# HPCForge/Bubbleformer

Measured on AMD Instinct MI355X. Metric: train samples/sec, FiLMAViT 16x192x192x4ch, bs=8 per GPU, higher is better.
Workload: dtype bf16; 1 GPU; FiLMAViT-small (E=384, 6 heads, 12 blocks, P=16, 9 fluid params) fwd + relative-L2 loss + bwd + AdamW, 4-field 16x192x192 clips, batch 8 per GPU (BASELINE.json configs[1]); global_batch=8, parallelism=dp1

## Files before the change

bubbleformer_amd/_lib.py:

```python
import ctypes as C
import os
import subprocess

_HERE = os.path.dirname(os.path.abspath(__file__))
LIB_PATH = os.path.join(_HERE, "libbubbleformer_hip.so")
CSRC = os.path.join(_HERE, "csrc")

BF_DTYPE_F32, BF_DTYPE_BF16 = 0, 1
BF_LAY_KC, BF_LAY_XC = 0, 1
BF_PRO_NONE, BF_PRO_AFFINE, BF_PRO_AFFINE_GELU, BF_PRO_GELU = 0, 1, 2, 3
BF_AUX_NONE, BF_AUX_ADD, BF_AUX_DGELU = 0, 1, 2
BF_OUT_STORE, BF_OUT_STORE_F32, BF_OUT_ATOMIC_F32 = 0, 1, 2
BF_MAX_STAGES = 5
BF_LOSS_LIMBS = 5

vp, fp, i32, i64, f32 = C.c_void_p, C.c_void_p, C.c_int32, C.c_int64, C.c_float


class Operand(C.Structure):
    _fields_ = [("p", vp), ("ld", i64), ("layout", i32), ("seglen", i32), ("segstride", i64), ("gw", i32), ("gh", i32),
                ("gc", i32), ("pro", i32), ("sc", fp), ("sh", fp), ("rows_per_frame", i32), ("nch", i32)]


class Epilogue(C.Structure):
# ... 4 lines not shown

class Dims(C.Structure):
    _fields_ = [(n, i32) for n in ("dtype", "B", "T", "h", "w", "E", "heads", "attn_scale", "feat_scale", "patch", "cin",
                                   "cout", "nfluid")]


TEMPORAL_FIELDS = ("gamma", "attn_scale_factor", "norm1_w", "norm1_b", "norm2_w", "norm2_b", "input_head_w", "input_head_b",
                   "output_head_w", "output_head_b", "qnorm_w", "qnorm_b", "knorm_w", "knorm_b", "rel_pos_emb")
SPATIAL_FIELDS = ("gamma_att", "gamma_mlp", "attn_scale_factor_x", "attn_scale_factor_y", "low_freq_scalar",
                  "high_freq_scalar", "norm1_w", "norm1_b", "norm2_w", "norm2_b", "input_head_w", "input_head_b",
                  "output_head_w", "output_head_b", "qnorm_w", "qnorm_b", "knorm_w", "knorm_b", "rel_pos_emb", "fc1_w", "fc1_b",
                  "fc2_w", "fc2_b", "mlp_norm_w", "mlp_norm_b")


class TemporalParams(C.Structure):
    _fields_ = [(n, fp) for n in TEMPORAL_FIELDS]


class SpatialParams(C.Structure):
    _fields_ = [(n, fp) for n in SPATIAL_FIELDS]


class FrameNorm(C.Structure):
    _fields_ = [("w", fp), ("b", fp), ("g", fp), ("gdiv", i32), ("mean", fp), ("rstd", fp), ("sc", fp), ("sh", fp), ("resid", vp), ("out", vp)]


class EmbedParams(C.Structure):
    _fields_ = [("conv_w", fp * BF_MAX_STAGES), ("in_w", fp * BF_MAX_STAGES), ("in_b", fp * BF_MAX_STAGES), ("film_ln_w", fp),
                ("film_ln_b", fp), ("film_w", fp), ("film_b", fp)]


class DebedParams(C.Structure):
    _fields_ = [("conv_w", fp * BF_MAX_STAGES), ("in_w", fp * BF_MAX_STAGES), ("in_b", fp * BF_MAX_STAGES)]


class ConvSrc(C.Structure):
    _fields_ = [("p", vp), ("C", i32), ("nchw", i32), ("f32", i32)]


class ConvGeo(C.Structure):
    _fields_ = [(n, i32) for n in ("F", "Hi", "Wi", "Ho", "Wo", "kh", "kw", "stride", "pad")]


BF_CONV_PRO_NONE, BF_CONV_PRO_AFFINE_GELU, BF_CONV_PRO_GELU = 0, 1, 2

STAGE_DONE_FN = C.CFUNCTYPE(None, C.c_int, C.c_void_p)
P = C.POINTER
SIGNATURES = {
    "bf_last_error": (C.c_char_p, []),
    "bf_abi_version": (C.c_int, []),
    "bf_prof_enable": (None, [C.c_int]),
    "bf_debug_force_generic_attn": (None, [C.c_int]),
    "bf_debug_tokred_fold": (None, [C.c_int]),
    "bf_side_defer": (None, [C.c_int]),
    "bf_prep_stages": (C.c_int, [C.POINTER(Dims), C.c_int, C.POINTER(C.c_int32), C.POINTER(vp), C.POINTER(vp), C.POINTER(vp), vp]),
    "bf_stage_prepared": (None, [C.c_int]),
    "bf_trunk_train_fwd": (C.c_int, [C.POINTER(Dims), C.c_int, C.POINTER(C.c_int32), C.POINTER(vp), C.POINTER(vp), C.POINTER(vp), C.POINTER(vp), vp,
                                     C.POINTER(vp), vp, vp]),
    "bf_trunk_train_bwd": (C.c_int, [C.POINTER(Dims), C.c_int, C.POINTER(C.c_int32), C.POINTER(vp), C.POINTER(vp), C.POINTER(vp), C.POINTER(vp),
                                     C.POINTER(vp), vp, C.POINTER(vp), vp, C.POINTER(vp), vp, vp, vp, vp, vp]),
    "bf_field_stats_ws_doubles": (i64, [C.c_int]),
    "bf_field_stats": (C.c_int, [fp, vp, vp, C.c_int, vp, vp, vp]),
    "bf_stage_chain_next": (C.c_int, [C.POINTER(Dims), C.c_int, vp, vp]),
    "bf_stage_next_scale": (C.c_int, [fp, C.c_int]),
    "bf_gemm_fwd_frames": (C.c_int, [C.c_int, C.c_int, C.c_int, C.c_int, vp, i64, vp, i64, fp, fp, fp, fp, C.c_int, vp, vp, C.c_int,
                                     C.POINTER(FrameNorm), C.POINTER(FrameNorm), vp]),
    "bf_trunk_eval_weights_bytes": (i64, [C.POINTER(Dims), C.c_int, C.POINTER(C.c_int32)]),
    "bf_trunk_eval_prepare": (C.c_int, [C.POINTER(Dims), C.c_int, C.POINTER(C.c_int32), C.POINTER(vp), vp, vp]),
    "bf_trunk_eval_fwd": (C.c_int, [C.POINTER(Dims), C.c_int, C.POINTER(C.c_int32), C.POINTER(vp), vp, vp, vp, vp, vp]),
    "bf_frame_linear": (C.c_int, [C.c_int, C.c_int, C.c_int, C.c_int, C.c_int, vp, i64, vp, i64, fp, fp, fp, fp, fp, vp, i64, C.c_int, fp, fp, fp,
                                  vp, i64, fp, fp, vp, i64, vp]),
    "bf_side_join": (C.c_int, [vp]),
    "bf_prof_report": (C.c_int, [C.c_char_p, C.c_int]),
    "bf_gemm": (C.c_int, [C.c_int, C.c_int, C.c_int, C.c_int, P(Operand), P(Operand), P(Epilogue), C.c_int, vp]),
    "bf_gemm_tokred": (C.c_int, [C.c_int, C.c_int, C.c_int, i64, vp, i64, vp, i64, fp, C.c_int, fp, fp, i64, vp]),
    "bf_gemm_tokred_ws_floats": (i64, [C.c_int, C.c_int, i64]),
    "bf_gemm_inbwd_frames": (C.c_int, [C.c_int, C.c_int, C.c_int, C.c_int, vp, i64, vp, i64, vp, vp, vp, C.c_int, fp, fp, fp, fp, fp, C.c_int, vp]),
    "bf_gemm_inbwd_frames_chain": (C.c_int, [C.c_int, C.c_int, C.c_int, C.c_int, vp, i64, vp, i64, vp, vp, vp, C.c_int, fp, fp, fp, fp, fp, C.c_int,
                                             vp, vp, fp, fp, fp, fp, C.c_int, fp, vp]),
    "bf_in_stats": (C.c_int, [C.c_int, vp, C.c_int, C.c_int, C.c_int, fp, fp, fp, C.c_int, fp, fp, fp, fp, fp, fp, vp]),
    "bf_in_ws_floats": (i64, [C.c_int, C.c_int, C.c_int, C.c_int]),
    "bf_affine_apply": (C.c_int, [C.c_int, vp, vp, fp, fp, vp, i64, C.c_int, C.c_int, vp]),
    "bf_in_bwd": (C.c_int, [C.c_int, vp, vp, vp, vp, C.c_int, C.c_int, C.c_int, fp, fp, fp, fp, fp, C.c_int, C.c_int, fp, fp,
                            fp, fp, fp, vp]),
    "bf_colsum": (C.c_int, [C.c_int, vp, i64, C.c_int, fp, fp, vp]),
    "bf_attn_axial_fwd": (C.c_int, [C.c_int, vp, vp, i64, C.c_int, C.c_int, C.c_int, C.c_int, fp, fp, fp, fp, fp, fp, fp, vp]),
    "bf_attn_axial_norm_fwd": (C.c_int, [C.c_int, vp, vp, vp, i64, C.c_int, C.c_int, C.c_int, C.c_int, fp, fp, fp, fp, fp, fp, fp, fp, fp, fp, fp, fp,
                                         fp, vp]),
    "bf_attn_fwd": (C.c_int, [C.c_int, vp, vp, i64, C.c_int, i64, i64, i64, i64, C.c_int, C.c_int, fp, fp, fp, fp, fp, fp, f32,
                              C.c_int, vp]),
    "bf_attn_bwd": (C.c_int, [C.c_int, vp, vp, vp, i64, C.c_int, i64, i64, i64, i64, C.c_int, C.c_int, fp, fp, fp, fp, fp, fp,
                              fp, fp, fp, fp, fp, fp, f32, C.c_int, fp, i64, vp]),
    "bf_im2col_nchw": (C.c_int, [C.c_int, fp, vp, C.c_int, C.c_int, C.c_int, C.c_int, C.c_int, vp]),
    "bf_col2im_nchw": (C.c_int, [C.c_int, vp, fp, C.c_int, C.c_int, C.c_int, C.c_int, C.c_int, vp]),
    "bf_pm2nchw": (C.c_int, [fp, fp, fp, fp, C.c_int, C.c_int, C.c_int, C.c_int, C.c_int, vp]),
    "bf_debed_last_bwd": (C.c_int, [C.c_int, fp, fp, fp, fp, fp, vp, vp, vp, C.c_int, C.c_int, C.c_int, C.c_int, C.c_int, C.c_int, vp]),
    "bf_debed_last_bwd_norm": (C.c_int, [C.c_int, fp, fp, fp, fp, fp, vp, vp, vp, fp, fp, fp, fp, vp, fp, fp, C.c_int, C.c_int, C.c_int, C.c_int, C.c_int,
                                         C.c_int, fp, C.c_int64, vp]),
    "bf_gather_gemm": (C.c_int, [C.c_int, vp, vp, C.c_int, fp, fp, vp, C.c_int, C.c_int, C.c_int, C.c_int, C.c_int, vp]),
    "bf_scatter_gemm": (C.c_int, [C.c_int, vp, vp, C.c_int, fp, fp, vp, fp, C.c_int, C.c_int, C.c_int, C.c_int, C.c_int, vp]),
    "bf_gather_wgrad_ws_floats": (C.c_int64, [C.c_int, C.c_int, C.c_int]),
    "bf_gather_wgrad": (C.c_int, [C.c_int, vp, vp, fp, fp, fp, fp, fp, C.c_int, C.c_int, C.c_int, C.c_int, C.c_int, C.c_int, fp, C.c_int64, vp]),
    "bf_gather_gemm_rebuilt": (C.c_int, [C.c_int, vp, vp, vp, C.c_int, fp, fp, vp, C.c_int, C.c_int, C.c_int, C.c_int, C.c_int, vp]),
    "bf_gather_wgrad_rebuilt": (C.c_int, [C.c_int, vp, vp, vp, fp, fp, fp, C.c_int, C.c_int, C.c_int, C.c_int, C.c_int, C.c_int, fp, C.c_int64, vp]),
    "bf_stage_chain_head": (C.c_int, [vp, vp, vp]),
    "bf_stage_chain_tail": (C.c_int, [vp, vp, C.c_int]),
# ... 118 lines not shown
```

bubbleformer_amd/csrc/bf_common.h:

```cpp
#pragma once
#include <hip/hip_runtime.h>
#include <stdint.h>
#include <math.h>

#include "../../include/bubbleformer_hip.h"

typedef __bf16 bf16;
typedef __attribute__((ext_vector_type(8))) __bf16 bf16x8;
typedef __attribute__((ext_vector_type(4))) __bf16 bf16x4;
typedef __attribute__((ext_vector_type(4))) short s16x4;
typedef __attribute__((ext_vector_type(4))) float f32x4;

#define BF_WAVE 64
#define BF_IN_EPS 1e-5f

#define BF_CHECK_LAUNCH()                                   \
    do {                                                    \
        hipError_t e__ = hipGetLastError();                 \
        if (e__ != hipSuccess) return bf_fail(e__, __FILE__, __LINE__); \
    } while (0)
#define BF_REQUIRE(cond, msg)                                \
    do {                                                     \
        if (!(cond)) return bf_fail_msg(msg, __FILE__, __LINE__); \
    } while (0)
// ... 40 lines not shown
    bool& flag() { int dev = 0; (void)hipGetDevice(&dev); return done[(dev >= 0 && dev < 64) ? dev : 0]; }
};
template <class T> struct BfPerDevice {
    T tab[64] = {};
    T& get() { int dev = 0; (void)hipGetDevice(&dev); return tab[(dev >= 0 && dev < 64) ? dev : 0]; }
};
int bf_fail(hipError_t e, const char* file, int line);
int bf_fail_msg(const char* msg, const char* file, int line);
int bf_decline(const char* msg);

__device__ __forceinline__ float to_f(float x) { return x; }
__device__ __forceinline__ float to_f(bf16 x) { return (float)x; }
template <typename T> __device__ __forceinline__ T from_f(float x);
template <> __device__ __forceinline__ float from_f<float>(float x) { return x; }
template <> __device__ __forceinline__ bf16 from_f<bf16>(float x) { return (bf16)x; }

template <typename T> struct Chunk;
template <> struct Chunk<float> {
    static constexpr int N = 4;
    float4 raw;
    __device__ __forceinline__ void load(const float* p) { raw = *reinterpret_cast<const float4*>(p); }
    __device__ __forceinline__ void store(float* p) const { *reinterpret_cast<float4*>(p) = raw; }
    __device__ __forceinline__ void zero() { raw = make_float4(0.f, 0.f, 0.f, 0.f); }
    __device__ __forceinline__ float get(int i) const { return i == 0 ? raw.x : i == 1 ? raw.y : i == 2 ? raw.z : raw.w; }
    __device__ __forceinline__ void set(int i, float v) { if (i == 0) raw.x = v; else if (i == 1) raw.y = v; else if (i == 2) raw.z = v; else raw.w = v; }
};
template <> struct Chunk<bf16> {
    static constexpr int N = 8;
    bf16x8 raw;
    __device__ __forceinline__ void load(const bf16* p) { raw = *reinterpret_cast<const bf16x8*>(p); }
    __device__ __forceinline__ void store(bf16* p) const { *reinterpret_cast<bf16x8*>(p) = raw; }
    __device__ __forceinline__ void zero() { for (int i = 0; i < 8; ++i) raw[i] = (bf16)0.f; }
    __device__ __forceinline__ float get(int i) const { return (float)raw[i]; }
    __device__ __forceinline__ void set(int i, float v) { raw[i] = (bf16)v; }
};

__device__ __forceinline__ float erf_fast(float x) {
    const float ax = fabsf(x);
    const float t = __builtin_amdgcn_rcpf(1.0f + 0.3275911f * ax);
    const float poly = t * (0.254829592f + t * (-0.284496736f + t * (1.421413741f + t * (-1.453152027f + t * 1.061405429f))));
    const float r = 1.0f - poly * __expf(-ax * ax);
    return copysignf(r, x);
}
__device__ __forceinline__ float gelu_f(float x) { return 0.5f * x * (1.0f + erf_fast(x * 0.70710678118654752440f)); }
__device__ __forceinline__ float dgelu_f(float x) {
    const float ax = fabsf(x) * 0.70710678118654752440f;
    const float t = __builtin_amdgcn_rcpf(1.0f + 0.3275911f * ax);
    const float poly = t * (0.254829592f + t * (-0.284496736f + t * (1.421413741f + t * (-1.453152027f + t * 1.061405429f))));
    const float e = __expf(-0.5f * x * x);
    const float cdf = 0.5f * (1.0f + copysignf(1.0f - poly * e, x));
    return cdf + x * (0.39894228040143267794f * e);
}

__device__ __forceinline__ float phi_fast(float x) {
    const float xc = fminf(fmaxf(x, -4.0f), 4.0f), u = xc * xc;
    float r = -1.520480094e-09f;
    r = r * u + 1.180964698e-07f; r = r * u - 4.014221545e-06f; r = r * u + 7.960997465e-05f; r = r * u - 1.041295800e-03f;
    r = r * u + 9.641715296e-03f; r = r * u - 6.614117438e-02f; r = r * u + 3.988329119e-01f;
    return 0.5f + xc * r;
}
__device__ __forceinline__ float gelu_fast(float x) { return x * phi_fast(x); }
__device__ __forceinline__ float dgelu_fast(float x) {
    const float xc = fminf(fmaxf(x, -4.0f), 4.0f), u = xc * xc;
    float r = 9.387459194e-10f;
    r = r * u - 7.941240515e-08f; r = r * u + 2.950722870e-06f; r = r * u - 6.380590451e-05f; r = r * u + 8.975979855e-04f;
    r = r * u - 8.669717964e-03f; r = r * u + 5.833777581e-02f; r = r * u - 2.646917422e-01f; r = r * u + 7.975648121e-01f;
    return 0.5f + xc * r;
}

template <typename T> __device__ __forceinline__ float gelu_t(float x) { if constexpr (sizeof(T) == 2) return gelu_fast(x); else return gelu_f(x); }
template <typename T> __device__ __forceinline__ float dgelu_t(float x) { if constexpr (sizeof(T) == 2) return dgelu_fast(x); else return dgelu_f(x); }

template <class T> __device__ __forceinline__ T wave_sum(T v) {
#pragma unroll
    for (int o = 32; o > 0; o >>= 1) v += __shfl_xor(v, o, 64);
    return v;
}
__device__ __forceinline__ float wave_max(float v) {
#pragma unroll
    for (int o = 32; o > 0; o >>= 1) v = fmaxf(v, __shfl_xor(v, o, 64));
    return v;
}

static inline int bf_cdiv(long a, long b) { return (int)((a + b - 1) / b); }
static inline size_t bf_esize(int dtype) { return dtype == BF_DTYPE_BF16 ? 2 : 4; }
```

bubbleformer_amd/csrc/gemm_stream.hip:

```cpp
#include "gemm_common.h"
#include <stdio.h>
#include <stdlib.h>
#include <algorithm>

namespace {
using namespace bfgemm;

constexpr int BM = 256, BNB = 128, BK = 64;
constexpr int CHUNK = BNB * BK;
constexpr int ACHUNK = BM * BK;
constexpr int NSLOT = 2;

struct StreamArgs {
    const bf16* A; long lda; const bf16* W; long ldw; bf16* C; long ldc;
    const float* bias; const float* colscale; const float* colshift; const float* rowscale; int rpg;
    int aux_mode; const bf16* aux; long ld_aux; bf16* gelu_out;
    int KS, mt, nb, ng;
    int mh, hunit;
    int stagger;
    int dbg;
};

__device__ __forceinline__ void wait_vm_n(int n) {
    if (n >= 16) { wait_vm<16>(); return; }
    switch (n) {
        case 0: wait_vm<0>(); break;   case 1: wait_vm<1>(); break;   case 2: wait_vm<2>(); break;   case 3: wait_vm<3>(); break;
        case 4: wait_vm<4>(); break;   case 5: wait_vm<5>(); break;   case 6: wait_vm<6>(); break;   case 7: wait_vm<7>(); break;
        case 8: wait_vm<8>(); break;   case 9: wait_vm<9>(); break;   case 10: wait_vm<10>(); break; case 11: wait_vm<11>(); break;
        case 12: wait_vm<12>(); break; case 13: wait_vm<13>(); break; case 14: wait_vm<14>(); break; default: wait_vm<15>(); break;
    }
}
__device__ __forceinline__ void gload16(uint4& dst, const void* p) { asm volatile("global_load_dwordx4 %0, %1, off" : "=v"(dst) : "v"(p) : "memory"); }

__device__ __forceinline__ void gload4(float& dst, const void* p) { asm volatile("global_load_dword %0, %1, off" : "=v"(dst) : "v"(p) : "memory"); }

template <int AUX, bool GELU2, bool CS>
__global__ void __launch_bounds__(512) stream_gemm_kernel(StreamArgs a) {
    extern __shared__ __attribute__((aligned(16))) char smem[];
    bf16* Bres = reinterpret_cast<bf16*>(smem);
    bf16* ring = Bres + (size_t)a.KS * CHUNK;
    const int KS = a.KS;
    const int tid = threadIdx.x, lane = tid & 63, wave = __builtin_amdgcn_readfirstlane(tid >> 6);
    const int wm = wave >> 1, wn = wave & 1;

    const int xl = blockIdx.x & 7, j = blockIdx.x >> 3, wpx = gridDim.x >> 3;
    const int tpx = wpx / a.nb;
    if (j >= tpx * a.nb) return;
    const int team = xl * tpx + j / a.nb, nteams = 8 * tpx;
    const int grp = team % a.ng, rank = team / a.ng, gteams = (nteams - grp + a.ng - 1) / a.ng;
    const int c_nb = grp * a.nb + j % a.nb;
    const int h_beg = a.hunit * (int)((long)(a.mh / a.hunit) * rank / gteams), h_end = a.hunit * (int)((long)(a.mh / a.hunit) * (rank + 1) / gteams);
    if (h_beg >= h_end) return;
    const int ntile = (h_end - h_beg + 1) >> 1;
    const bool odd_run = (h_end - h_beg) & 1;
    const int total_steps = ntile * KS;

    long roffA[4], roffB[2];
#pragma unroll
    for (int t = 0; t < 4; ++t) {
        const int r = 8 * (wave * 4 + t) + (lane >> 3);
        roffA[t] = (long)r * a.lda + 8 * ((lane & 7) ^ ((r >> 1) & 7));
    }
#pragma unroll
    for (int t = 0; t < 2; ++t) {
        const int r = 8 * (wave * 2 + t) + (lane >> 3);
        roffB[t] = (long)r * a.ldw + 8 * ((lane & 7) ^ ((r >> 1) & 7));
    }
    const unsigned lds0 = lds_addr(smem);
    const unsigned ldsB = __builtin_amdgcn_readfirstlane(lds0 + (unsigned)wave * 2048u);
    const unsigned ldsA = __builtin_amdgcn_readfirstlane(lds0 + (unsigned)KS * (unsigned)(CHUNK * 2) + (unsigned)wave * 4096u);

    int issued = 0;
    int i_ks = 0, i_left = total_steps, i_slot = 0;
    const bf16* i_row = a.A + (long)((a.dbg & 2) ? 0 : h_beg) * (BM / 2) * a.lda;
    auto issue_A = [&]() {
        const unsigned dst = ldsA + (unsigned)i_slot * (unsigned)(ACHUNK * 2);
        if (!(odd_run && i_left <= KS && wave >= 4)) {
#pragma unroll
            for (int t = 0; t < 4; ++t) glds16(i_row + roffA[t] + i_ks * BK, dst + t * 1024u);
            issued += 4;
        }
        i_slot ^= 1;
        --i_left;
        if (++i_ks == KS) { i_ks = 0; if (!(a.dbg & 2)) i_row += (long)BM * a.lda; }
    };

    const int li = lane & 15, lg = lane >> 4;
    const int c8 = wn * 64 + (lg & 1) * 16 + (lg >> 1) * 8;
    float e_bias[2][8], e_cs[2][CS ? 8 : 1], e_ch[2][CS ? 8 : 1];
    {
#pragma unroll
        for (int pp = 0; pp < 2; ++pp)
#pragma unroll
            for (int q = 0; q < 8; ++q) {
                const int n = c_nb * BNB + c8 + 32 * pp + q;
                e_bias[pp][q] = a.bias ? a.bias[n] : 0.f;
                if constexpr (CS) { e_cs[pp][q] = a.colscale ? a.colscale[n] : 1.f; e_ch[pp][q] = a.colscale ? a.colshift[n] : 0.f; }
            }
#pragma unroll
        for (int pp = 0; pp < 2; ++pp)
#pragma unroll
            for (int q = 0; q < 8; ++q) {
                asm volatile("" : "+v"(e_bias[pp][q]));
                if constexpr (CS) { asm volatile("" : "+v"(e_cs[pp][q])); asm volatile("" : "+v"(e_ch[pp][q])); }
            }
    }

    int bmark[6];
    const bf16* w0 = a.W + (long)c_nb * BNB * a.ldw;
    auto load_W = [&](int kb) {
#pragma unroll
        for (int t = 0; t < 2; ++t) glds16(w0 + roffB[t] + kb * BK, ldsB + (unsigned)kb * (unsigned)(CHUNK * 2) + t * 1024u);
        issued += 2;
        return issued;
    };
    bmark[0] = load_W(0);
    issue_A();
    int mark = issued, mark_next = issued;
    bmark[1] = load_W(1);
    const bool pre1 = i_left > 0;
    if (pre1) { issue_A(); mark_next = issued; }
#pragma unroll
    for (int kb = 2; kb < 6; ++kb) bmark[kb] = kb < KS ? load_W(kb) : issued;
    bool first_tile = true;

    f32x4 acc[4][4];
    uint4 auxr[4][2];
    float rsr[4] = {1.f, 1.f, 1.f, 1.f};
    const bool has_rs = CS && a.rowscale != nullptr;
    int aux_mark = 0;
    int slot = 0;
    auto run_tile = [&](int tt) __attribute__((always_inline)) {
        const int m0 = h_beg * (BM / 2) + tt * BM;
#pragma unroll
        for (int i = 0; i < 4; ++i)
#pragma unroll
            for (int jn = 0; jn < 4; ++jn) acc[i][jn] = f32x4{0.f, 0.f, 0.f, 0.f};
        for (int ks = 0; ks < KS; ++ks) {
            int need = mark;
            if (first_tile) { const int bm = ks == 0 ? bmark[0] : ks == 1 ? bmark[1] : ks == 2 ? bmark[2] : ks == 3 ? bmark[3] : ks == 4 ? bmark[4] : bmark[5]; need = max(need, bm); }
            if (!(a.dbg & 1)) wait_vm_n(issued - need);
            asm volatile("s_waitcnt lgkmcnt(0)" ::: "memory");
            __builtin_amdgcn_s_barrier();
            if (ks == 0) {
                if constexpr (AUX != BF_AUX_NONE) {
#pragma unroll
                    for (int i = 0; i < 4; ++i)
#pragma unroll
                        for (int pp = 0; pp < 2; ++pp)
                            gload16(auxr[i][pp], a.aux + (long)(m0 + wm * 64 + i * 16 + li) * a.ld_aux + c_nb * BNB + c8 + 32 * pp);
                    issued += 8;
                }
                if (has_rs) {
#pragma unroll
                    for (int i = 0; i < 4; ++i) gload4(rsr[i], a.rowscale + (m0 + wm * 64 + i * 16 + li) / a.rpg);
                    issued += 4;
                }
                aux_mark = issued;
            }
            const bool late = a.stagger && wave >= 4;
            const bool skip = first_tile && ks == 0 && pre1;
            if (!late && !skip) { if (i_left > 0 && !(a.dbg & 32)) issue_A(); mark_next = issued; }
            const bf16* cA = ring + (size_t)slot * ACHUNK;
            const bf16* cB = Bres + (size_t)ks * CHUNK;
            if (!(a.dbg & 4))
#pragma unroll
            for (int kk = 0; kk < BK; kk += 32) {
                if (kk == 32 && late && !skip) { if (i_left > 0 && !(a.dbg & 32)) issue_A(); mark_next = issued; }
                bf16x8 fa[4], fb[4];
#pragma unroll
                for (int i = 0; i < 4; ++i) fa[i] = frag_bf16<false, BK>(cA, wm * 64 + i * 16, kk, lane);
#pragma unroll
                for (int jn = 0; jn < 4; ++jn) fb[jn] = frag_bf16<false, BK>(cB, wn * 64 + jn * 16, kk, lane);
#pragma unroll
                for (int i = 0; i < 4; ++i)
#pragma unroll
                    for (int jn = 0; jn < 4; ++jn) acc[i][jn] = __builtin_amdgcn_mfma_f32_16x16x32_bf16(fb[jn], fa[i], acc[i][jn], 0, 0, 0);
            }
            slot ^= 1;
            mark = mark_next;
        }
        first_tile = false;
        if (AUX != BF_AUX_NONE || has_rs) {
            wait_vm_n(issued - aux_mark);
            if constexpr (AUX != BF_AUX_NONE) {
#pragma unroll
                for (int i = 0; i < 4; ++i)
#pragma unroll
                    for (int pp = 0; pp < 2; ++pp) asm volatile("" : "+v"(auxr[i][pp].x), "+v"(auxr[i][pp].y), "+v"(auxr[i][pp].z), "+v"(auxr[i][pp].w));
            }
            if constexpr (CS) {
#pragma unroll
                for (int i = 0; i < 4; ++i) asm volatile("" : "+v"(rsr[i]));
            }
            __builtin_amdgcn_sched_barrier(0);
        }
#pragma unroll
        for (int i = 0; i < 4; ++i) {
            const int m = m0 + wm * 64 + i * 16 + li;
#pragma unroll
            for (int pp = 0; pp < 2; ++pp) {
                float v[8];
#pragma unroll
                for (int r = 0; r < 4; ++r) {
                    typedef __attribute__((ext_vector_type(2))) unsigned u32x2;
                    const u32x2 sw = __builtin_amdgcn_permlane16_swap(__float_as_uint(acc[i][2 * pp][r]), __float_as_uint(acc[i][2 * pp + 1][r]), false, false);
                    v[r] = __uint_as_float(sw[0]); v[4 + r] = __uint_as_float(sw[1]);
                }
                if constexpr (AUX == BF_AUX_ADD) {
                    const bf16x8 ax = __builtin_bit_cast(bf16x8, auxr[i][pp]);
#pragma unroll
                    for (int q = 0; q < 8; ++q) {
                        float cs_ = 1.f, ch_ = 0.f;
                        if constexpr (CS) { cs_ = e_cs[pp][q]; ch_ = e_ch[pp][q]; }
                        v[q] = epi_lin_add(v[q], e_bias[pp][q], cs_, ch_, has_rs ? rsr[i] : 1.f, CS, (float)ax[q]);
                    }
                } else {
#pragma unroll
                    for (int q = 0; q < 8; ++q) {
                        float cs_ = 1.f, ch_ = 0.f;
                        if constexpr (CS) { cs_ = e_cs[pp][q]; ch_ = e_ch[pp][q]; }
                        v[q] = epi_lin(v[q], e_bias[pp][q], cs_, ch_, has_rs ? rsr[i] : 1.f, CS);
                    }
                    if constexpr (AUX == BF_AUX_DGELU) {
                        const bf16x8 ax = __builtin_bit_cast(bf16x8, auxr[i][pp]);
#pragma unroll
                        for (int q = 0; q < 8; ++q) v[q] = v[q] * dgelu_fast((float)ax[q]);
                    }
                }
                bf16x8 o;
#pragma unroll
                for (int q = 0; q < 8; ++q) o[q] = (bf16)v[q];
                const long off = (long)m * a.ldc + c_nb * BNB + c8 + 32 * pp;
                if (a.dbg & 16) asm volatile("" :: "v"(o)); else
                if (!(a.dbg & 8)) *reinterpret_cast<bf16x8*>(a.C + off) = o;
                if constexpr (GELU2) {
                    bf16x8 g8;
#pragma unroll
                    for (int q = 0; q < 8; ++q) g8[q] = (bf16)gelu_fast(v[q]);
                    *reinterpret_cast<bf16x8*>(a.gelu_out + off) = g8;
                }
            }
        }
        issued += GELU2 ? 16 : 8;
    };
    const int nfull = odd_run ? ntile - 1 : ntile;
    for (int tt = 0; tt < nfull; ++tt) run_tile(tt);
    if (odd_run) {
        if (wave < 4) run_tile(ntile - 1);
        else
            for (int ks = 0; ks < KS; ++ks) {
                wait_vm<0>();
                asm volatile("s_waitcnt lgkmcnt(0)" ::: "memory");
                __builtin_amdgcn_s_barrier();
            }
    }
}


constexpr int PSLOT = (ACHUNK + CHUNK) * 2;
constexpr int PNSLOT = 3;

__device__ __forceinline__ void wait_vm_wide(int n) {
    if (n < 16) { wait_vm_n(n); return; }
    if (n >= 40) { wait_vm<40>(); return; }
    switch ((n - 16) >> 2) {
        case 0: wait_vm<16>(); break; case 1: wait_vm<20>(); break; case 2: wait_vm<24>(); break;
        case 3: wait_vm<28>(); break; case 4: wait_vm<32>(); break; default: wait_vm<36>(); break;
    }
}

template <int AUX, bool GELU2, bool CS>
__global__ void __launch_bounds__(512) stream_pp_kernel(StreamArgs a) {
    extern __shared__ __attribute__((aligned(16))) char smem[];
    const int KS = a.KS;
    const int tid = threadIdx.x, lane = tid & 63, wave = __builtin_amdgcn_readfirstlane(tid >> 6);
    const int wm = wave >> 1, wn = wave & 1;
    const bool late = wave >= 4;

    const int xl = blockIdx.x & 7, j = blockIdx.x >> 3, wpx = gridDim.x >> 3;
    const int tpx = wpx / a.nb;
    if (j >= tpx * a.nb) return;
    const int team = xl * tpx + j / a.nb, nteams = 8 * tpx;
    const int grp = team % a.ng, rank = team / a.ng, gteams = (nteams - grp + a.ng - 1) / a.ng;
    const int c_nb = grp * a.nb + j % a.nb;
    const int t_beg = (int)((long)a.mt * rank / gteams), t_end = (int)((long)a.mt * (rank + 1) / gteams);
    if (t_beg >= t_end) return;
    const int total_steps = (t_end - t_beg) * KS;

    long roffA[4], roffB[2];
#pragma unroll
    for (int t = 0; t < 4; ++t) {
        const int r = 8 * (wave * 4 + t) + (lane >> 3);
        roffA[t] = (long)r * a.lda + 8 * ((lane & 7) ^ ((r >> 1) & 7));
    }
#pragma unroll
    for (int t = 0; t < 2; ++t) {
        const int r = 8 * (wave * 2 + t) + (lane >> 3);
        roffB[t] = (long)r * a.ldw + 8 * ((lane & 7) ^ ((r >> 1) & 7));
    }
    const unsigned lds0 = lds_addr(smem);
    const unsigned ldsA = __builtin_amdgcn_readfirstlane(lds0 + (unsigned)wave * 4096u);
    const unsigned ldsB = __builtin_amdgcn_readfirstlane(lds0 + (unsigned)(ACHUNK * 2) + (unsigned)wave * 2048u);
    const bf16* w0 = a.W + (long)c_nb * BNB * a.ldw;

    int issued = 0;
    int i_ks = 0, i_left = total_steps, i_slot = 0;
    const bf16* i_row = a.A + (long)t_beg * BM * a.lda;
    auto issue_lo = [&]() {
// ... 153 lines not shown
                        float cs_ = 1.f, ch_ = 0.f;
                        if constexpr (CS) { cs_ = e_cs[pp][q]; ch_ = e_ch[pp][q]; }
                        v[q] = epi_lin(v[q], e_bias[pp][q], cs_, ch_, has_rs ? rsr[i] : 1.f, CS);
                    }
                    if constexpr (AUX == BF_AUX_DGELU) {
                        const bf16x8 ax = __builtin_bit_cast(bf16x8, auxr[i][pp]);
#pragma unroll
                        for (int q = 0; q < 8; ++q) v[q] = v[q] * dgelu_fast((float)ax[q]);
                    }
                }
                bf16x8 o;
#pragma unroll
                for (int q = 0; q < 8; ++q) o[q] = (bf16)v[q];
                const long off = (long)m * a.ldc + c_nb * BNB + c8 + 32 * pp;
                *reinterpret_cast<bf16x8*>(a.C + off) = o;
                if constexpr (GELU2) {
                    bf16x8 g8;
#pragma unroll
                    for (int q = 0; q < 8; ++q) g8[q] = (bf16)gelu_fast(v[q]);
                    *reinterpret_cast<bf16x8*>(a.gelu_out + off) = g8;
                }
            }
        }
        issued += GELU2 ? 16 : 8;
    }
}


int num_cus() {
    static const int n = []() {
        int dev = 0; hipDeviceProp_t p;
        if (hipGetDevice(&dev) != hipSuccess || hipGetDeviceProperties(&p, dev) != hipSuccess || p.multiProcessorCount < 8) return 256;
        return p.multiProcessorCount;
    }();
    return n;
}

bool team_split(int NB, int mt, int wpx, int* nb, int* ng) {
    static const int force = bf_knob("BF_STREAM_GROUPS", 0);
    int best = 0, best_cost = 0;
    for (int g = 1; g <= NB; ++g) {
        if (NB % g || NB / g > wpx || (force > 0 && g != force)) continue;
        const int nteams = 8 * (wpx / (NB / g));
        if (nteams < g) continue;
        const int fewest = nteams / g;
        const int cost = (mt + fewest - 1) / fewest;
        if (!best || cost < best_cost) { best = g; best_cost = cost; }
    }
    if (!best) return false;
    *ng = best; *nb = NB / best;
    return true;
}

}

int bf_gemm_stream_try(int M, int N, int K, const bf_operand* A, const bf_operand* B, const bf_epilogue* E, hipStream_t st) {
    static const int enabled = bf_knob("BF_GEMM_STREAM", 1);
    if (!enabled) return 1;
    if (A->layout != BF_LAY_KC || B->layout != BF_LAY_KC || A->pro != BF_PRO_NONE || B->pro != BF_PRO_NONE) return 1;
    if (A->gw > 0 || A->seglen > 0 || B->gw > 0 || B->seglen > 0 || E->gw > 0 || E->seglen > 0) return 1;
    if (E->out_mode != BF_OUT_STORE || E->colsum) return 1;
    static const int pp_env = bf_knob("BF_STREAM_PP", -1);
    if (M % BM || N % BNB || K % BK || K < 2 * BK) return 1;
    const bool ws_ok = K >= 4 * BK && K <= 6 * BK;
    const bool use_pp = pp_env == 1 || !ws_ok;
    if (pp_env == 0 && !ws_ok) return 1;
    if (A->ld % 8 || B->ld % 8 || E->ldc % 8 || (E->aux_mode != BF_AUX_NONE && E->ld_aux % 8)) return 1;
    if (((uintptr_t)A->p | (uintptr_t)B->p | (uintptr_t)E->c | (uintptr_t)E->aux | (uintptr_t)E->gelu_out) & 15) return 1;
    if (E->gelu_out && E->aux_mode != BF_AUX_NONE) return 1;
    if (E->colscale && !E->colshift) return 1;
    StreamArgs a;
    a.A = (const bf16*)A->p; a.lda = A->ld; a.W = (const bf16*)B->p; a.ldw = B->ld; a.C = (bf16*)E->c; a.ldc = E->ldc;
    a.bias = E->bias; a.colscale = E->colscale; a.colshift = E->colshift; a.rowscale = E->rowscale; a.rpg = E->rows_per_group > 0 ? E->rows_per_group : 1;
    a.aux_mode = E->aux_mode; a.aux = (const bf16*)E->aux; a.ld_aux = E->ld_aux; a.gelu_out = (bf16*)E->gelu_out;
    a.KS = K / BK; a.mt = M / BM; a.mh = M / (BM / 2);
    static const int half_on = bf_knob("BF_STREAM_HALF", 1);
    a.hunit = half_on ? 1 : 2;
    const int grid = (num_cus() / 8) * 8;
    if (!team_split(N / BNB, (use_pp || !half_on) ? a.mt : a.mh, grid / 8, &a.nb, &a.ng)) return 1;
    static const int dbg = bf_knob("BF_STREAM_DEBUG", 0);
    a.dbg = dbg;
    static const int stagger = bf_knob("BF_STREAM_STAGGER", 1);
    a.stagger = stagger;
    const int lds_bytes = a.KS * CHUNK * 2 + NSLOT * ACHUNK * 2;
    static thread_local char pname[64];
    snprintf(pname, sizeof(pname), use_pp ? "stream_pp<%s>" : "stream_gemm<%s>", E->gelu_out ? "gelu2" : E->aux_mode == BF_AUX_ADD ? "add" : E->aux_mode == BF_AUX_DGELU ? "dgelu" : "plain");
    BfProfScope prof(st, pname, 2.0 * M * N * K, ((double)M * K + (double)N * K + (double)M * N * (E->gelu_out ? 2 : 1) + (E->aux_mode != BF_AUX_NONE ? (double)M * N : 0.0)) * 2.0);
#define BF_STREAM_GO(AUXM, G2, CSF)                                                                                                       \
    do {                                                                                                                                \
        static BfPerDeviceOnce attr_once, attr_pp_once; bool& attr_done = attr_once.flag(); bool& attr_pp_done = attr_pp_once.flag();                                                                            \
        if (use_pp) {                                                                                                                   \
            if (!attr_pp_done) {                                                                                                        \
                hipError_t e_ = hipFuncSetAttribute((const void*)stream_pp_kernel<AUXM, G2, CSF>, hipFuncAttributeMaxDynamicSharedMemorySize, PNSLOT * PSLOT); \
                if (e_ != hipSuccess) return bf_fail(e_, __FILE__, __LINE__);                                                           \
                attr_pp_done = true;                                                                                                    \
            }                                                                                                                           \
            hipLaunchKernelGGL((stream_pp_kernel<AUXM, G2, CSF>), dim3(grid), dim3(512), PNSLOT * PSLOT, st, a);                        \
            break;                                                                                                                      \
        }                                                                                                                               \
        if (!attr_done) {                                                                                                               \
            hipError_t e_ = hipFuncSetAttribute((const void*)stream_gemm_kernel<AUXM, G2, CSF>, hipFuncAttributeMaxDynamicSharedMemorySize, 6 * CHUNK * 2 + NSLOT * ACHUNK * 2); \
            if (e_ != hipSuccess) return bf_fail(e_, __FILE__, __LINE__);                                                               \
            attr_done = true;                                                                                                           \
        }                                                                                                                               \
        hipLaunchKernelGGL((stream_gemm_kernel<AUXM, G2, CSF>), dim3(grid), dim3(512), lds_bytes, st, a);                                    \
    } while (0)
    const bool cs = E->colscale != nullptr || E->rowscale != nullptr;
    if (E->gelu_out && !cs) BF_STREAM_GO(BF_AUX_NONE, true, false);
    else if (E->gelu_out) return 1;
    else if (E->aux_mode == BF_AUX_ADD && cs) BF_STREAM_GO(BF_AUX_ADD, false, true);
    else if (E->aux_mode == BF_AUX_ADD) BF_STREAM_GO(BF_AUX_ADD, false, false);
    else if (E->aux_mode == BF_AUX_DGELU && !cs) BF_STREAM_GO(BF_AUX_DGELU, false, false);
    else if (E->aux_mode == BF_AUX_DGELU) return 1;
    else if (cs) return 1;
    else BF_STREAM_GO(BF_AUX_NONE, false, false);
#undef BF_STREAM_GO
    BF_CHECK_LAUNCH();
    return 0;
}
```

include/bubbleformer_hip.h:

```cpp
#ifndef BUBBLEFORMER_HIP_H
#define BUBBLEFORMER_HIP_H

#include <stdint.h>

#ifdef __cplusplus
extern "C" {
#endif

typedef void* bf_stream_t;

enum { BF_DTYPE_F32 = 0, BF_DTYPE_BF16 = 1 };

enum { BF_LAY_KC = 0,
       BF_LAY_XC = 1   };
enum { BF_PRO_NONE = 0, BF_PRO_AFFINE = 1, BF_PRO_AFFINE_GELU = 2, BF_PRO_GELU = 3 };
enum { BF_AUX_NONE = 0, BF_AUX_ADD = 1 , BF_AUX_DGELU = 2  };
enum { BF_OUT_STORE = 0 , BF_OUT_ATOMIC_F32 = 2 ,
       BF_OUT_STORE_F32 = 1  };

typedef struct bf_operand {
    const void* p;
    int64_t ld;
    int32_t layout;
    int32_t seglen;
// ... 44 lines not shown
    const void* resid;
    void* out;
} bf_frame_norm;
int bf_gemm_fwd_frames(int dtype, int M, int N, int K, const void* A, int64_t lda, const void* Bt, int64_t ldb, const float* bias,
                       const float* colscale, const float* colshift, const float* fscale, int fdiv, const void* add, void* out, int S,
                       const bf_frame_norm* n1, const bf_frame_norm* n2, bf_stream_t stream);

int bf_gemm_tokred(int dtype, int Nout, int Kin, int64_t M, const void* dy, int64_t ldy, const void* x, int64_t ldx, float* out,
                   int accumulate, float* colsum, float* ws, int64_t ws_floats, bf_stream_t stream);
int64_t bf_gemm_tokred_ws_floats(int Nout, int Kin, int64_t M);

int bf_frame_linear(int dtype, int frames, int S, int K, int N, const void* A, int64_t lda, const void* W, int64_t ldw,
                    const float* norm_w, const float* norm_b, const float* bias, const float* colscale, const float* colshift,
                    const void* resid, int64_t ldr, int gelu, const float* en_w, const float* en_b, const float* en_g,
                    void* out, int64_t ldo,
                    const float* next_w, const float* next_b, void* out_n, int64_t ldn,
                    bf_stream_t stream);


int bf_in_stats(int dtype, const void* x, int frames, int S, int C, const float* w, const float* b, const float* g, int gdiv,
                const float* gb, float* mean, float* rstd, float* sc, float* sh,
                float* ws ,
                bf_stream_t stream);
int64_t bf_in_ws_floats(int dtype, int frames, int S, int C);
int bf_affine_apply(int dtype, const void* z, const void* resid, const float* sc, const float* sh, void* out, int64_t nrows,
                    int S, int C, bf_stream_t stream);
int bf_in_bwd(int dtype, const void* dy, const void* x, const void* add, void* dx, int frames, int S, int C, const float* mean,
              const float* rstd, const float* w, const float* b, const float* g, int gdiv, int gelu, float* dw, float* db,
              float* dg, float* dgb, float* ws ,
              bf_stream_t stream);
int bf_colsum(int dtype, const void* x, int64_t nrows, int C, const float* scale, float* out, bf_stream_t stream);

int bf_attn_fwd(int dtype, const void* qkv, void* out, int64_t nseq, int L, int64_t inner, int64_t outer_stride,
                int64_t inner_stride, int64_t tok_stride, int heads, int d, const float* qw, const float* qb, const float* kw,
                const float* kb, const float* emb, const float* hscale, float out_scale, int accumulate, bf_stream_t stream);
int bf_attn_axial_fwd(int dtype, const void* qkv, void* out, int64_t frames, int h, int w, int heads, int d, const float* qw,
                      const float* qb, const float* kw, const float* kb, const float* emb, const float* hscale_x,
                      const float* hscale_y, bf_stream_t stream);
int bf_attn_axial_norm_fwd(int dtype, const void* qkv, void* out, void* out_n, int64_t frames, int h, int w, int heads, int d,
                           const float* qw, const float* qb, const float* kw, const float* kb, const float* emb, const float* hscale_x,
                           const float* hscale_y, const float* norm_w, const float* norm_b, float* mean, float* rstd, float* sc,
                           float* sh, bf_stream_t stream);
int bf_attn_bwd(int dtype, const void* qkv, const void* dout, void* dqkv, int64_t nseq, int L, int64_t inner,
                int64_t outer_stride, int64_t inner_stride, int64_t tok_stride, int heads, int d, const float* qw,
                const float* qb, const float* kw, const float* kb, const float* emb, const float* hscale, float* dqw,
                float* dqb, float* dkw, float* dkb, float* demb, float* dhscale, float out_scale, int accumulate,
                float* ws, int64_t ws_floats,
                bf_stream_t stream);

void bf_side_defer(int on);
int bf_side_join(bf_stream_t stream);
void bf_debug_force_generic_attn(int on);
void bf_debug_tokred_fold(int on);

int bf_im2col_nchw(int dtype, const float* x, void* out, int frames, int C, int H, int W, int Kp, bf_stream_t stream);
int bf_col2im_nchw(int dtype, const void* g, float* dx, int frames, int C, int H, int W, int Kp, bf_stream_t stream);
#define BF_LOSS_LIMBS 5
int bf_pm2nchw(const float* pm, float* pred, const float* y, float* lossbuf, int frames, int Co, int h, int w, int Np,
               bf_stream_t stream);
int bf_debed_last(int dtype, const void* act, const float* sc, const float* sh, const void* wc, float* pred, const float* y,
                  float* lossbuf, int frames, int Ci, int Co, int h, int w, int Np, bf_stream_t stream);
int bf_debed_last_bwd(int dtype, const float* dpred, const float* pred, const float* y, const float* coef, const float* gscale,
                      const void* wc, void* dpm, void* dact, int frames, int Ci, int Co, int h, int w, int Np, bf_stream_t stream);
int bf_debed_last_bwd_norm(int dtype, const float* dpred, const float* pred, const float* y, const float* coef, const float* gscale,
                           const void* wc, void* dpm, const void* ymap, const float* mean, const float* rstd, const float* in_w,
                           const float* in_b, void* dx, float* d_in_w, float* d_in_b, int frames, int Ci, int Co, int h, int w, int Np,
                           float* ws, int64_t ws_floats, bf_stream_t stream);
int bf_embed_first(int dtype, const float* x, const void* wc, void* patches, void* y0, int frames, int C0, int cin, int h2, int w2,
                   int Kp, float* stat_part, bf_stream_t stream);
int bf_in_stats_merge_slices(int dtype, int frames, int S, int C, int rows, const float* w, const float* b, const float* g, int gdiv,
                             const float* gb, float* mean, float* rstd, float* sc, float* sh, float* ws, bf_stream_t stream);
int bf_gather_gemm(int dtype, const void* map, const void* w, int w_kn, const float* sc, const float* sh, void* out, int frames, int gh,
                   int gw, int C0, int N, bf_stream_t stream);
int bf_scatter_gemm(int dtype, const void* a, const void* w, int w_kn, const float* sc, const float* sh, void* map, float* stat_part, int frames,
                    int gh, int gw, int K, int C0, bf_stream_t stream);
int64_t bf_gather_wgrad_ws_floats(int frames, int gh, int gw);
int bf_gather_wgrad(int dtype, const void* fine, const void* coarse, const float* fsc, const float* fsh, const float* csc, const float* csh,
                    float* out, int transposed, int frames, int gh, int gw, int C0, int Kc, float* ws, int64_t ws_floats, bf_stream_t stream);
int bf_gather_gemm_rebuilt(int dtype, const void* patches, const void* w0c, const void* w, int w_kn, const float* sc, const float* sh, void* out,
                           int frames, int gh, int gw, int C0, int N, bf_stream_t stream);
int bf_gather_wgrad_rebuilt(int dtype, const void* patches, const void* w0c, const void* coarse, const float* fsc, const float* fsh, float* out,
                            int transposed, int frames, int gh, int gw, int C0, int Kc, float* ws, int64_t ws_floats, bf_stream_t stream);
int64_t bf_embed_tail_ws_floats(int frames, int gh1, int gw1, int C0, int Kp);
int bf_embed_tail_bwd(int dtype, const void* dy1, const void* w1c, const void* y0, const void* patches, const void* w0c, const float* sc,
                      const float* sh, const float* mean, const float* rstd, const float* in_w, float* dwprep, float* d_in_w, float* d_in_b,
                      int frames, int gh1, int gw1, int C1, int C0, int Kp, float* ws, int64_t ws_floats, bf_stream_t stream);
int bf_lploss_finalize(const float* lossbuf, int frames, int Co, float* loss, float* coef, bf_stream_t stream);
int bf_nchw2pm(int dtype, const float* dpred, const float* pred, const float* y, const float* coef, const float* gscale,
               void* dpm, int frames, int Co, int h, int w, int Np, bf_stream_t stream);
int bf_wprep(int dtype, int mode, const float* src, void* dst, int R, int K, int Kp, bf_stream_t stream);
int bf_wgrad_unprep(int mode, const float* gsrc, float* gdst, int R, int K, int Kp, int transposed, bf_stream_t stream);
int bf_film_net_fwd(const float* cond, const float* lnw, const float* lnb, const float* W, const float* bias, float* gb,
                    float* chat, float* crstd, int B, int P, int E2, bf_stream_t stream);
int bf_film_net_bwd(const float* dgb, const float* chat, const float* lnw, const float* lnb, const float* W, float* dW,
                    float* dbias, float* dlnw, float* dlnb, int B, int P, int E2, bf_stream_t stream);
int bf_adamw(float* p, const float* g, float* m, float* v, int64_t n, int step, float lr, float beta1, float beta2, float eps,
             float wd, float gscale, bf_stream_t stream);
int bf_adam(float* p, const float* g, float* m, float* v, int64_t n, int step, float lr, float beta1, float beta2, float eps,
            float wd, float gscale, bf_stream_t stream);
int bf_clip_gather(const float* src, int64_t field_stride, const int32_t* field, const int64_t* first, int t0, const float* diff,
                   const float* div, float* out, int B, int T, int C, int H, int W, int Ho, int Wo, bf_stream_t stream);
int bf_clip_gather_batch(const float* src, int64_t field_stride, const int64_t* idx, int64_t nsamples, const int64_t* first_tab, const int32_t* in_field,
                         const float* in_diff, const float* in_div, int Cin, int Tin, float* in_out, const int32_t* out_field,
                         const float* out_diff, const float* out_div, int Cout, int Tout, float* out_out, const float* fluid_tab,
                         const int64_t* file_tab, int P, float* fluid_out, int B, int H, int W, int Ho, int Wo, bf_stream_t stream);
int64_t bf_field_stats_ws_doubles(int nseg);
// ... 166 lines not shown
```

Measured before the change: 823.6 samples/s.

## Phase-stagger stream GEMM wave groups and pack GELU polynomials into paired floats

```diff
diff --git a/bubbleformer_amd/_lib.py b/bubbleformer_amd/_lib.py
--- a/bubbleformer_amd/_lib.py
+++ b/bubbleformer_amd/_lib.py
@@ -80,6 +80,7 @@
     "bf_prof_enable": (None, [C.c_int]),
     "bf_debug_force_generic_attn": (None, [C.c_int]),
     "bf_debug_tokred_fold": (None, [C.c_int]),
+    "bf_debug_stream_phase": (None, [C.c_int]),
     "bf_side_defer": (None, [C.c_int]),
     "bf_prep_stages": (C.c_int, [C.POINTER(Dims), C.c_int, C.POINTER(C.c_int32), C.POINTER(vp), C.POINTER(vp), C.POINTER(vp), vp]),
     "bf_stage_prepared": (None, [C.c_int]),
diff --git a/bubbleformer_amd/csrc/bf_common.h b/bubbleformer_amd/csrc/bf_common.h
--- a/bubbleformer_amd/csrc/bf_common.h
+++ b/bubbleformer_amd/csrc/bf_common.h
@@ -116,21 +116,49 @@
     return cdf + x * (0.39894228040143267794f * e);
 }
 
-__device__ __forceinline__ float phi_fast(float x) {
-    const float xc = fminf(fmaxf(x, -4.0f), 4.0f), u = xc * xc;
-    float r = -1.520480094e-09f;
-    r = r * u + 1.180964698e-07f; r = r * u - 4.014221545e-06f; r = r * u + 7.960997465e-05f; r = r * u - 1.041295800e-03f;
-    r = r * u + 9.641715296e-03f; r = r * u - 6.614117438e-02f; r = r * u + 3.988329119e-01f;
-    return 0.5f + xc * r;
+template <int N, int NC> __device__ __forceinline__ void odd_poly_half_n(const float (&x)[N], float (&out)[N], const float (&c)[NC]) {
+    if constexpr (N == 1) {
+        const float xc = fminf(fmaxf(x[0], -4.0f), 4.0f), u = xc * xc;
+        float r = c[0];
+#pragma unroll
+        for (int k = 1; k < NC; ++k) r = r * u + c[k];
+        out[0] = 0.5f + xc * r;
+    } else {
+        static_assert(N == 8, "pairs of four");
+        typedef float f32x2 __attribute__((ext_vector_type(2)));
+        f32x2 xc[4], u[4], r[4];
+#pragma unroll
+        for (int p = 0; p < 4; ++p) {
+            xc[p] = f32x2{fminf(fmaxf(x[2 * p], -4.0f), 4.0f), fminf(fmaxf(x[2 * p + 1], -4.0f), 4.0f)};
+            u[p] = xc[p] * xc[p];
+            r[p] = f32x2{c[0], c[0]};
+        }
+#pragma unroll
+        for (int k = 1; k < NC; ++k) {
+#pragma unroll
+            for (int p = 0; p < 4; ++p) r[p] = r[p] * u[p] + f32x2{c[k], c[k]};
+            asm volatile("" : "+v"(r[0]), "+v"(r[1]), "+v"(r[2]), "+v"(r[3]));
+        }
+#pragma unroll
+        for (int p = 0; p < 4; ++p) {
+            const f32x2 o = f32x2{0.5f, 0.5f} + xc[p] * r[p];
+            out[2 * p] = o[0]; out[2 * p + 1] = o[1];
+        }
+    }
 }
+template <int N> __device__ __forceinline__ void phi_fast_n(const float (&x)[N], float (&out)[N]) {
+    constexpr float c[8] = {-1.520480094e-09f, 1.180964698e-07f, -4.014221545e-06f, 7.960997465e-05f, -1.041295800e-03f, 9.641715296e-03f,
+                            -6.614117438e-02f, 3.988329119e-01f};
+    odd_poly_half_n<N, 8>(x, out, c);
+}
+template <int N> __device__ __forceinline__ void dgelu_fast_n(const float (&x)[N], float (&out)[N]) {
+    constexpr float c[9] = {9.387459194e-10f, -7.941240515e-08f, 2.950722870e-06f, -6.380590451e-05f, 8.975979855e-04f, -8.669717964e-03f,
+                            5.833777581e-02f, -2.646917422e-01f, 7.975648121e-01f};
+    odd_poly_half_n<N, 9>(x, out, c);
+}
+__device__ __forceinline__ float phi_fast(float x) { const float a[1] = {x}; float o[1]; phi_fast_n<1>(a, o); return o[0]; }
 __device__ __forceinline__ float gelu_fast(float x) { return x * phi_fast(x); }
-__device__ __forceinline__ float dgelu_fast(float x) {
-    const float xc = fminf(fmaxf(x, -4.0f), 4.0f), u = xc * xc;
-    float r = 9.387459194e-10f;
-    r = r * u - 7.941240515e-08f; r = r * u + 2.950722870e-06f; r = r * u - 6.380590451e-05f; r = r * u + 8.975979855e-04f;
-    r = r * u - 8.669717964e-03f; r = r * u + 5.833777581e-02f; r = r * u - 2.646917422e-01f; r = r * u + 7.975648121e-01f;
-    return 0.5f + xc * r;
-}
+__device__ __forceinline__ float dgelu_fast(float x) { const float a[1] = {x}; float o[1]; dgelu_fast_n<1>(a, o); return o[0]; }
 
 template <typename T> __device__ __forceinline__ float gelu_t(float x) { if constexpr (sizeof(T) == 2) return gelu_fast(x); else return gelu_f(x); }
 template <typename T> __device__ __forceinline__ float dgelu_t(float x) { if constexpr (sizeof(T) == 2) return dgelu_fast(x); else return dgelu_f(x); }
diff --git a/bubbleformer_amd/csrc/gemm_stream.hip b/bubbleformer_amd/csrc/gemm_stream.hip
--- a/bubbleformer_amd/csrc/gemm_stream.hip
+++ b/bubbleformer_amd/csrc/gemm_stream.hip
@@ -18,6 +18,7 @@
     int KS, mt, nb, ng;
     int mh, hunit;
     int stagger;
+    int phase;
     int dbg;
 };
 
@@ -33,6 +34,12 @@
 __device__ __forceinline__ void gload16(uint4& dst, const void* p) { asm volatile("global_load_dwordx4 %0, %1, off" : "=v"(dst) : "v"(p) : "memory"); }
 
 __device__ __forceinline__ void gload4(float& dst, const void* p) { asm volatile("global_load_dword %0, %1, off" : "=v"(dst) : "v"(p) : "memory"); }
+
+constexpr int NE = 2;
+constexpr bool slice_start(int g) {
+    for (int s = 1; s < NE; ++s) if (8 * s / NE == g) return true;
+    return false;
+}
 
 template <int AUX, bool GELU2, bool CS>
 __global__ void __launch_bounds__(512) stream_gemm_kernel(StreamArgs a) {
@@ -130,18 +137,37 @@
     const bool has_rs = CS && a.rowscale != nullptr;
     int aux_mark = 0;
     int slot = 0;
+    int gi = 0;
+    auto w_need = [&](int g) { return g == 0 ? bmark[0] : g == 1 ? bmark[1] : g == 2 ? bmark[2] : g == 3 ? bmark[3] : g == 4 ? bmark[4] : g == 5 ? bmark[5] : 0; };
+    auto arrive = [&](int n) {
+        for (int k = 0; k < n; ++k) {
+            if (gi < 6) wait_vm_n(issued - w_need(gi));
+            asm volatile("s_waitcnt lgkmcnt(0)" ::: "memory");
+            __builtin_amdgcn_s_barrier();
+            ++gi;
+        }
+    };
+    auto slice_barrier = [&]() __attribute__((always_inline)) {
+        if (a.phase) {
+            __builtin_amdgcn_sched_barrier(0);
+            __builtin_amdgcn_s_barrier();
+            __builtin_amdgcn_sched_barrier(0);
+            ++gi;
+        }
+    };
     auto run_tile = [&](int tt) __attribute__((always_inline)) {
         const int m0 = h_beg * (BM / 2) + tt * BM;
 #pragma unroll
         for (int i = 0; i < 4; ++i)
 #pragma unroll
             for (int jn = 0; jn < 4; ++jn) acc[i][jn] = f32x4{0.f, 0.f, 0.f, 0.f};
+        if (a.phase) __builtin_amdgcn_s_setprio(1);
         for (int ks = 0; ks < KS; ++ks) {
-            int need = mark;
-            if (first_tile) { const int bm = ks == 0 ? bmark[0] : ks == 1 ? bmark[1] : ks == 2 ? bmark[2] : ks == 3 ? bmark[3] : ks == 4 ? bmark[4] : bmark[5]; need = max(need, bm); }
+            const int need = max(mark, w_need(gi));
             if (!(a.dbg & 1)) wait_vm_n(issued - need);
             asm volatile("s_waitcnt lgkmcnt(0)" ::: "memory");
             __builtin_amdgcn_s_barrier();
+            ++gi;
             if (ks == 0) {
                 if constexpr (AUX != BF_AUX_NONE) {
 #pragma unroll
@@ -181,6 +207,8 @@
             mark = mark_next;
         }
         first_tile = false;
+        if (a.phase) __builtin_amdgcn_s_setprio(0);
+        slice_barrier();
         if (AUX != BF_AUX_NONE || has_rs) {
             wait_vm_n(issued - aux_mark);
             if constexpr (AUX != BF_AUX_NONE) {
@@ -200,6 +228,7 @@
             const int m = m0 + wm * 64 + i * 16 + li;
 #pragma unroll
             for (int pp = 0; pp < 2; ++pp) {
+                if (slice_start(2 * i + pp)) slice_barrier();
                 float v[8];
 #pragma unroll
                 for (int r = 0; r < 4; ++r) {
@@ -224,8 +253,12 @@
                     }
                     if constexpr (AUX == BF_AUX_DGELU) {
                         const bf16x8 ax = __builtin_bit_cast(bf16x8, auxr[i][pp]);
-#pragma unroll
-                        for (int q = 0; q < 8; ++q) v[q] = v[q] * dgelu_fast((float)ax[q]);
+                        float x8[8], d8[8];
+#pragma unroll
+                        for (int q = 0; q < 8; ++q) x8[q] = (float)ax[q];
+                        dgelu_fast_n<8>(x8, d8);
+#pragma unroll
+                        for (int q = 0; q < 8; ++q) v[q] = v[q] * d8[q];
                     }
                 }
                 bf16x8 o;
@@ -236,25 +269,21 @@
                 if (!(a.dbg & 8)) *reinterpret_cast<bf16x8*>(a.C + off) = o;
                 if constexpr (GELU2) {
                     bf16x8 g8;
-#pragma unroll
-                    for (int q = 0; q < 8; ++q) g8[q] = (bf16)gelu_fast(v[q]);
+                    float p8[8];
+                    phi_fast_n<8>(v, p8);
+#pragma unroll
+                    for (int q = 0; q < 8; ++q) g8[q] = (bf16)(v[q] * p8[q]);
                     *reinterpret_cast<bf16x8*>(a.gelu_out + off) = g8;
                 }
             }
         }
         issued += GELU2 ? 16 : 8;
     };
-    const int nfull = odd_run ? ntile - 1 : ntile;
-    for (int tt = 0; tt < nfull; ++tt) run_tile(tt);
-    if (odd_run) {
-        if (wave < 4) run_tile(ntile - 1);
-        else
-            for (int ks = 0; ks < KS; ++ks) {
-                wait_vm<0>();
-                asm volatile("s_waitcnt lgkmcnt(0)" ::: "memory");
-                __builtin_amdgcn_s_barrier();
-            }
-    }
+    const int mine = (odd_run && wave >= 4) ? ntile - 1 : ntile;
+    const int lead = a.phase ? NE : 0;
+    if (wave >= 4) arrive(lead);
+    for (int tt = 0; tt < mine; ++tt) run_tile(tt);
+    arrive((ntile - mine) * (KS + lead) + (wave < 4 ? lead : 0));
 }
 
 
@@ -514,7 +543,11 @@
     return true;
 }
 
-}
+int g_stream_phase = -1;
+
+}
+
+extern "C" void bf_debug_stream_phase(int phase) { g_stream_phase = phase < 0 ? -1 : (phase != 0); }
 
 int bf_gemm_stream_try(int M, int N, int K, const bf_operand* A, const bf_operand* B, const bf_epilogue* E, hipStream_t st) {
     static const int enabled = bf_knob("BF_GEMM_STREAM", 1);
@@ -544,6 +577,7 @@
     a.dbg = dbg;
     static const int stagger = bf_knob("BF_STREAM_STAGGER", 1);
     a.stagger = stagger;
+    a.phase = g_stream_phase >= 0 ? g_stream_phase : (E->gelu_out != nullptr || E->aux_mode == BF_AUX_DGELU);
     const int lds_bytes = a.KS * CHUNK * 2 + NSLOT * ACHUNK * 2;
     static thread_local char pname[64];
     snprintf(pname, sizeof(pname), use_pp ? "stream_pp<%s>" : "stream_gemm<%s>", E->gelu_out ? "gelu2" : E->aux_mode == BF_AUX_ADD ? "add" : E->aux_mode == BF_AUX_DGELU ? "dgelu" : "plain");
diff --git a/include/bubbleformer_hip.h b/include/bubbleformer_hip.h
--- a/include/bubbleformer_hip.h
+++ b/include/bubbleformer_hip.h
@@ -120,6 +120,7 @@
 int bf_side_join(bf_stream_t stream);
 void bf_debug_force_generic_attn(int on);
 void bf_debug_tokred_fold(int on);
+void bf_debug_stream_phase(int phase);
 
 int bf_im2col_nchw(int dtype, const float* x, void* out, int frames, int C, int H, int W, int Kp, bf_stream_t stream);
 int bf_col2im_nchw(int dtype, const void* g, float* dx, int frames, int C, int H, int W, int Kp, bf_stream_t stream);
```

Result: slower. 808.6 samples/s (-1.8%).
